# halajun/VDO_SLAM

Measured on AMD Instinct MI355X. Metric: frames/sec (per-frame hot path, KITTI-0000-shaped 1242x375) + ms/LM-iter (batch factor graph), higher is better.
Workload: dtype f64 (LM, RANSAC) / u8,i32,f32 (front-end, tracking)

## Files before the change

vdo_slam_amd/csrc/near_flags.hpp:

```cpp
#pragma once
#include <hip/hip_runtime.h>
#include <stdint.h>

namespace vdo {

static __global__ __launch_bounds__(256) void k_near_flags(int nq, const float* __restrict__ qx, const float* __restrict__ qy,
                                                           int nr, const float* __restrict__ rx, const float* __restrict__ ry, int32_t* __restrict__ used) {
  __shared__ float sx[256], sy[256];
  const int i = blockIdx.x * 256 + threadIdx.x;
  const int base = blockIdx.y * 256;
  const int j = base + threadIdx.x;
  sx[threadIdx.x] = j < nr ? rx[j] : 1e30f;
  sy[threadIdx.x] = j < nr ? ry[j] : 1e30f;
  __syncthreads();
  if (i >= nq) return;
  const float x = qx[i], y = qy[i];
  const int m = min(256, nr - base);
  int u = 0;
  for (int k = 0; k < m; ++k) {
    const float dx = sx[k] - x, dy = sy[k] - y;
    if (dx * dx + dy * dy < 1.0f) u = 1;
  }
  if (u) atomicOr(&used[i], 1);
}

static __global__ __launch_bounds__(256) void k_near_flags_sel(int nq, const float* __restrict__ qx, const float* __restrict__ qy,
                                                               int nr, const float* __restrict__ rx, const float* __restrict__ ry,
                                                               const int32_t* __restrict__ rsel, int as_int, int32_t* __restrict__ used) {
  __shared__ float sx[256], sy[256];
  const int i = blockIdx.x * 256 + threadIdx.x;
  const int base = blockIdx.y * 256;
  const int j = base + threadIdx.x;
  float vx = 1e30f, vy = 1e30f;
  if (j < nr && rsel[j]) { vx = rx[j]; vy = ry[j]; if (as_int) { vx = (float)(int)vx; vy = (float)(int)vy; } }
  sx[threadIdx.x] = vx; sy[threadIdx.x] = vy;
  __syncthreads();
  if (i >= nq) return;
  const float x = qx[i], y = qy[i];
  const int m = min(256, nr - base);
  int u = 0;
  for (int k = 0; k < m; ++k) {
    const float dx = sx[k] - x, dy = sy[k] - y;
    if (dx * dx + dy * dy < 1.0f) u = 1;
  }
  if (u) atomicOr(&used[i], 1);
}
static inline void launch_near_flags_sel(hipStream_t s, int nq, const float* qx, const float* qy, int nr, const float* rx, const float* ry, const int32_t* rsel, int as_int, int32_t* used,
                                         bool zero = true) {
  if (zero) hipMemsetAsync(used, 0, sizeof(int32_t) * (size_t)nq, s);
  if (nq > 0 && nr > 0) hipLaunchKernelGGL(k_near_flags_sel, dim3((nq + 255) / 256, (nr + 255) / 256), dim3(256), 0, s, nq, qx, qy, nr, rx, ry, rsel, as_int, used);
}

static inline void launch_near_flags(hipStream_t s, int nq, const float* qx, const float* qy, int nr, const float* rx, const float* ry, int32_t* used) {
  hipMemsetAsync(used, 0, sizeof(int32_t) * (size_t)nq, s);
  if (nq > 0 && nr > 0) hipLaunchKernelGGL(k_near_flags, dim3((nq + 255) / 256, (nr + 255) / 256), dim3(256), 0, s, nq, qx, qy, nr, rx, ry, used);
}

}
```

vdo_slam_amd/csrc/tracking.hip:

```cpp
#include <algorithm>
#include <cstring>
#include <vector>

#include "../../include/vdo_slam_hip.h"
#include "ctx.hpp"
#include "frame_images.hpp"
#include "near_flags.hpp"
#include "arena.hpp"
#include "tracking_shared.hpp"

namespace vdo {

__global__ void k_gather(int mode, int n, const float* __restrict__ kx, const float* __restrict__ ky, const float* __restrict__ depth,
                         const int32_t* __restrict__ mask, int w, int h, float th, float* __restrict__ dout, int32_t* __restrict__ lout) {
  const int i = blockIdx.x * blockDim.x + threadIdx.x;
  if (i >= n) return;
  const int u = (int)kx[i], v = (int)ky[i];
  if (mode == 0) {
    float o = -1.f;
    if (u < (w - 1) && u > 0 && v < (h - 1) && v > 0) { const float d = depth[(size_t)v * w + u]; if (d > 0) o = d; }
    dout[i] = o;
  } else if (mode == 1) {
    float o = 0.1f; int l = 0;
    if (u < (w - 1) && u > 0 && v < (h - 1) && v > 0) {
      const float d = depth[(size_t)v * w + u];
      if (d < th && d > 0) { o = d; l = mask[(size_t)v * w + u]; }
    }
    dout[i] = o; lout[i] = l;
  } else {
    lout[i] = (u < w && u > 0 && v < h && v > 0) ? mask[(size_t)v * w + u] : -1;
  }
}


__global__ void k_get3d_world(int n, const float* __restrict__ kx, const float* __restrict__ ky, const float* __restrict__ d, Cam c, float* __restrict__ xyz) {
  const int i = blockIdx.x * blockDim.x + threadIdx.x;
  if (i >= n) return;
  float o[3];
  backproject(c, kx[i], ky[i], d[i], o);
  xyz[3 * i] = o[0]; xyz[3 * i + 1] = o[1]; xyz[3 * i + 2] = o[2];
}

__global__ void k_scene_flow(int n, const float* __restrict__ cx_, const float* __restrict__ cy_, const float* __restrict__ cd, const int32_t* __restrict__ cl, Cam cc,
                             const float* __restrict__ lx, const float* __restrict__ ly, const float* __restrict__ ld, const int32_t* __restrict__ ll, Cam lc,
                             float* __restrict__ flow3d, int32_t* __restrict__ objlab) {
  const int i = blockIdx.x * blockDim.x + threadIdx.x;
  if (i >= n) return;
  if (cl[i] <= 0 || ll[i] <= 0) { objlab[i] = -1; flow3d[3 * i] = 0; flow3d[3 * i + 1] = 0; flow3d[3 * i + 2] = 0; return; }
  float p[3], c[3];
  backproject(lc, lx[i], ly[i], ld[i], p);
  backproject(cc, cx_[i], cy_[i], cd[i], c);
  flow3d[3 * i] = c[0] - p[0]; flow3d[3 * i + 1] = c[1] - p[1]; flow3d[3 * i + 2] = c[2] - p[2];
}

__global__ void k_renew_pred(int n, const float* __restrict__ px, const float* __restrict__ py, const int32_t* __restrict__ mask,
                             const float* __restrict__ depth, const float* __restrict__ flow, int w, int h,
                             int32_t* __restrict__ ok, float* __restrict__ fx, float* __restrict__ fy, float* __restrict__ dout) {
  const int i = blockIdx.x * blockDim.x + threadIdx.x;
  if (i >= n) return;
  const float x_ = px[i], y_ = py[i];
  const int x = (int)x_, y = (int)y_;
  int good = 0;
  float fxe = 0, fye = 0, d = -1.f;
  if (!(x >= w || y >= h || x <= 0 || y <= 0)) {
    const size_t o = (size_t)y * w + x;
    const float dd = depth[o];
    if (mask[o] == 0 && !(dd > 40 || dd <= 0)) {
      fxe = flow[2 * o]; fye = flow[2 * o + 1];
      if (fxe != 0 && fye != 0 && x_ + fxe < w && y_ + fye < h && x_ + fxe > 0 && y_ + fye > 0) { good = 1; d = dd > 0 ? dd : -1.f; }
    }
  }
  ok[i] = good; fx[i] = fxe; fy[i] = fye; dout[i] = d;
}

__global__ __launch_bounds__(1024) void k_carry_select(int n, const int32_t* __restrict__ ok, int max_keep, int32_t* __restrict__ sel) {
  __shared__ int lds[17];
  int carry = 0;
  for (int base = 0; base < n; base += 1024) {
    const int i = base + threadIdx.x;
    const int v = (i < n && ok[i]) ? 1 : 0;
    const int lane = threadIdx.x & 63, wv = threadIdx.x >> 6;
    int incl = v;
#pragma unroll
    for (int off = 1; off < 64; off <<= 1) { const int t = __shfl_up(incl, off, 64); if (lane >= off) incl += t; }
    __syncthreads();
    if (lane == 63) lds[wv] = incl;
    __syncthreads();
    if (threadIdx.x == 0) { int a = 0; for (int q = 0; q < 16; ++q) { const int t = lds[q]; lds[q] = a; a += t; } lds[16] = a; }
    __syncthreads();
    const int rank = carry + lds[wv] + incl - v;
    if (i < n) sel[i] = (v && rank <= max_keep) ? 1 : 0;
    carry += lds[16];
    __syncthreads();
  }
}

__global__ void k_mask_warp(const int32_t* __restrict__ mask_last, const float* __restrict__ flow_last, int w, int h, int32_t lab, int32_t* __restrict__ mask_cur) {
  const int k = blockIdx.x * blockDim.x + threadIdx.x, j = blockIdx.y;
  if (k >= w) return;
  const size_t o = (size_t)j * w + k;
  if (mask_last[o] != lab) return;
  const int fx = (int)flow_last[2 * o], fy = (int)flow_last[2 * o + 1];
  if (k + fx < w && k + fx > 0 && j + fy < h && j + fy > 0) mask_cur[(size_t)(j + fy) * w + (k + fx)] = lab;
}

}

using namespace vdo;

extern "C" int vdo_propagate_static(vdo_frame_images* f, int n, const float* kx, const float* ky, float* depth_out) {
  if (!f || n < 0) return set_error(VDO_ERR_INVALID, "bad argument");
  if (n == 0) return VDO_OK;
  int rc = ctx_bind(f->ctx);
  if (rc != VDO_OK) return rc;
  Arena S(f->ctx);
  if (!S.reserve(Arena::bytes_for(3 * (size_t)n))) return set_error(VDO_ERR_OOM, "scratch arena: allocation failed");
  float *dx = S.up(kx, n), *dy = S.up(ky, n), *dd = S.up<float>(nullptr, n);
  if (!dd) return set_error(VDO_ERR_OOM, "hipMalloc failed");
  hipLaunchKernelGGL(k_gather, dim3((n + 255) / 256), dim3(256), 0, S.stream(), 0, n, (const float*)dx, (const float*)dy, (const float*)f->d_depth, (const int32_t*)f->d_mask, f->w, f->h, 0.f, dd, (int32_t*)nullptr);
  S.down(depth_out, dd, n);
  return S.finish("vdo_propagate_static");
}

extern "C" int vdo_propagate_object(vdo_frame_images* f, int n, const float* kx, const float* ky, float th_depth_obj, float* depth_out, int32_t* label_out) {
  if (!f || n < 0) return set_error(VDO_ERR_INVALID, "bad argument");
  if (n == 0) return VDO_OK;
  int rc = ctx_bind(f->ctx);
  if (rc != VDO_OK) return rc;
  Arena S(f->ctx);
  if (!S.reserve(Arena::bytes_for(4 * (size_t)n))) return set_error(VDO_ERR_OOM, "scratch arena: allocation failed");
  float *dx = S.up(kx, n), *dy = S.up(ky, n), *dd = S.up<float>(nullptr, n);
  int32_t* dl = S.up<int32_t>(nullptr, n);
  if (!dl) return set_error(VDO_ERR_OOM, "hipMalloc failed");
  hipLaunchKernelGGL(k_gather, dim3((n + 255) / 256), dim3(256), 0, S.stream(), 1, n, (const float*)dx, (const float*)dy, (const float*)f->d_depth, (const int32_t*)f->d_mask, f->w, f->h, th_depth_obj, dd, dl);
  S.down(depth_out, dd, n); S.down(label_out, dl, n);
  return S.finish("vdo_propagate_object");
}

extern "C" int vdo_mask_at(vdo_frame_images* f, int n, const float* cx, const float* cy, int32_t* label_out) {
  if (!f || n < 0) return set_error(VDO_ERR_INVALID, "bad argument");
  if (n == 0) return VDO_OK;
  int rc = ctx_bind(f->ctx);
  if (rc != VDO_OK) return rc;
  Arena S(f->ctx);
  if (!S.reserve(Arena::bytes_for(3 * (size_t)n))) return set_error(VDO_ERR_OOM, "scratch arena: allocation failed");
  float *dx = S.up(cx, n), *dy = S.up(cy, n);
  int32_t* dl = S.up<int32_t>(nullptr, n);
  if (!dl) return set_error(VDO_ERR_OOM, "hipMalloc failed");
  hipLaunchKernelGGL(k_gather, dim3((n + 255) / 256), dim3(256), 0, S.stream(), 2, n, (const float*)dx, (const float*)dy, (const float*)f->d_depth, (const int32_t*)f->d_mask, f->w, f->h, 0.f, (float*)nullptr, dl);
  S.down(label_out, dl, n);
  return S.finish("vdo_mask_at");
}

extern "C" int vdo_mask_warp(vdo_frame_images* cur, vdo_frame_images* last, int32_t label) {
  if (!cur || !last || cur->w != last->w || cur->h != last->h) return set_error(VDO_ERR_INVALID, "bad argument");
  int rc = ctx_bind(cur->ctx);
  if (rc != VDO_OK) return rc;
  hipLaunchKernelGGL(k_mask_warp, dim3((cur->w + 255) / 256, cur->h), dim3(256), 0, cur->ctx->stream, (const int32_t*)last->d_mask, (const float*)last->d_flow, cur->w, cur->h, label, cur->d_mask);
  return VDO_OK;
}

extern "C" int vdo_frame_images_download_mask(vdo_frame_images* f, int32_t* mask_out) {
  if (!f || !mask_out) return set_error(VDO_ERR_INVALID, "bad argument");
  int rc = ctx_bind(f->ctx);
  if (rc != VDO_OK) return rc;
  hipMemcpyAsync(mask_out, f->d_mask, 4 * (size_t)f->w * f->h, hipMemcpyDeviceToHost, f->ctx->stream);
  hipError_t e = hipStreamSynchronize(f->ctx->stream);
  if (e == hipSuccess) e = hipGetLastError();
  if (e != hipSuccess) return set_error(VDO_ERR_NO_DEVICE, "vdo_frame_images_download_mask: %s", hipGetErrorString(e));
  return VDO_OK;
}

extern "C" int vdo_frame_images_download_depth(vdo_frame_images* f, float* depth_out) {
  if (!f || !depth_out) return set_error(VDO_ERR_INVALID, "bad argument");
  int rc = ctx_bind(f->ctx);
  if (rc != VDO_OK) return rc;
  hipMemcpyAsync(depth_out, f->d_depth, 4 * (size_t)f->w * f->h, hipMemcpyDeviceToHost, f->ctx->stream);
  hipError_t e = hipStreamSynchronize(f->ctx->stream);
  if (e == hipSuccess) e = hipGetLastError();
  if (e != hipSuccess) return set_error(VDO_ERR_NO_DEVICE, "vdo_frame_images_download_depth: %s", hipGetErrorString(e));
  return VDO_OK;
}

extern "C" int vdo_frame_images_download_flow(vdo_frame_images* f, float* flow_out) {
  if (!f || !flow_out) return set_error(VDO_ERR_INVALID, "bad argument");
  int rc = ctx_bind(f->ctx);
  if (rc != VDO_OK) return rc;
  hipMemcpyAsync(flow_out, f->d_flow, 8 * (size_t)f->w * f->h, hipMemcpyDeviceToHost, f->ctx->stream);
  hipError_t e = hipStreamSynchronize(f->ctx->stream);
  if (e == hipSuccess) e = hipGetLastError();
  if (e != hipSuccess) return set_error(VDO_ERR_NO_DEVICE, "vdo_frame_images_download_flow: %s", hipGetErrorString(e));
  return VDO_OK;
}

extern "C" int vdo_get3d_world(vdo_ctx* ctx, int n, const float* kx, const float* ky, const float* depth, const float K4[4], const float Twc[16], float* xyz_out) {
  if (!ctx || n < 0) return set_error(VDO_ERR_INVALID, "bad argument");
  if (n == 0) return VDO_OK;
  int rc = ctx_bind(ctx);
  if (rc != VDO_OK) return rc;
  Arena S(ctx);
  if (!S.reserve(Arena::bytes_for(6 * (size_t)n))) return set_error(VDO_ERR_OOM, "scratch arena: allocation failed");
  float *dx = S.up(kx, n), *dy = S.up(ky, n), *dd = S.up(depth, n), *dxyz = S.up<float>(nullptr, 3 * (size_t)n);
  if (!dxyz) return set_error(VDO_ERR_OOM, "hipMalloc failed");
  hipLaunchKernelGGL(k_get3d_world, dim3((n + 255) / 256), dim3(256), 0, S.stream(), n, (const float*)dx, (const float*)dy, (const float*)dd, make_cam_Twc(K4, Twc), dxyz);
  S.down(xyz_out, dxyz, 3 * (size_t)n);
  return S.finish("vdo_get3d_world");
}

extern "C" int vdo_scene_flow(vdo_ctx* ctx, int n, const float* cur_x, const float* cur_y, const float* cur_d, const int32_t* cur_label, const float Tcw_cur[16],
                              const float* last_x, const float* last_y, const float* last_d, const int32_t* last_label, const float Tcw_last[16],
                              const float K4[4], float* flow3d_out, int32_t* obj_label_inout) {
  if (!ctx || n < 0) return set_error(VDO_ERR_INVALID, "bad argument");
  if (n == 0) return VDO_OK;
  int rc = ctx_bind(ctx);
  if (rc != VDO_OK) return rc;
  Arena S(ctx);
  if (!S.reserve(Arena::bytes_for(12 * (size_t)n))) return set_error(VDO_ERR_OOM, "scratch arena: allocation failed");
  float *a = S.up(cur_x, n), *b = S.up(cur_y, n), *c = S.up(cur_d, n), *d = S.up(last_x, n), *e = S.up(last_y, n), *g = S.up(last_d, n);
  int32_t *cl = S.up(cur_label, n), *ll = S.up(last_label, n), *ol = S.up(obj_label_inout, n);
  float* fl = S.up<float>(nullptr, 3 * (size_t)n);
  if (!fl) return set_error(VDO_ERR_OOM, "hipMalloc failed");
  hipLaunchKernelGGL(k_scene_flow, dim3((n + 255) / 256), dim3(256), 0, S.stream(), n, (const float*)a, (const float*)b, (const float*)c, (const int32_t*)cl, make_cam_Tcw(K4, Tcw_cur),
                     (const float*)d, (const float*)e, (const float*)g, (const int32_t*)ll, make_cam_Tcw(K4, Tcw_last), fl, ol);
  S.down(flow3d_out, fl, 3 * (size_t)n); S.down(obj_label_inout, ol, n);
  return S.finish("vdo_scene_flow");
}

namespace {
struct K9Args { float th_depth; int32_t* keep_idx; float *corr_x, *corr_y, *flow_x, *flow_y, *depth; int* n_out; };
}
static int renew_static_world_impl(vdo_frame_images* f, int n_tm, const int32_t* tm_sta, const float* stat_x, const float* stat_y,
                                   int n_orb, const float* orb_x, const float* orb_y, int max_num_sta, const float K4[4], const float Twc[16],
                                   float* key_x, float* key_y, float* corr_x, float* corr_y, float* flow_x, float* flow_y,
                                   int32_t* inlier_id, float* depth_out, float* xyz_out, int* n_out, const K9Args* k9) {
  if (!f || !n_out || n_tm < 0 || n_orb < 0 || (xyz_out && (!K4 || !Twc))) return set_error(VDO_ERR_INVALID, "bad argument");
  if (k9 && (!k9->n_out || 10 * (size_t)n_orb > 8 * (size_t)f->cap)) return set_error(VDO_ERR_INVALID, "bad argument / too many keypoints for the staging buffer");
  if (k9) *k9->n_out = 0;
  if (k9 && n_orb == 0) k9 = nullptr;
  int rc = ctx_bind(f->ctx);
  if (rc != VDO_OK) return rc;
  Arena S(f->ctx);
  if (!S.reserve(Arena::bytes_for(24 * ((size_t)n_tm + (size_t)n_orb) + 4 * (size_t)max_num_sta + (k9 ? 6 * (size_t)n_orb + 512 : 0)))) return set_error(VDO_ERR_OOM, "scratch arena: allocation failed");
  std::vector<float> cx1, cy1; std::vector<int32_t> id1;
  for (int i = 0; i < n_tm; ++i) if (tm_sta[i] != -1) { cx1.push_back(stat_x[tm_sta[i]]); cy1.push_back(stat_y[tm_sta[i]]); id1.push_back(tm_sta[i]); }
  const int n1 = (int)cx1.size();
  std::vector<int32_t> ok1(n1), ok2(n_orb), used2(n_orb, 0);
  std::vector<float> fx1(n1), fy1(n1), d1(n1), fx2(n_orb), fy2(n_orb), d2(n_orb), xyz1(xyz_out ? 3 * (size_t)n1 : 0), xyz2(xyz_out ? 3 * (size_t)n_orb : 0);
  float *dx1 = S.up(cx1.data(), n1), *dy1 = S.up(cy1.data(), n1);
  float *dx2 = S.up(orb_x, n_orb), *dy2 = S.up(orb_y, n_orb);
  int32_t *dok1 = S.up<int32_t>(nullptr, n1), *dsel1 = S.up<int32_t>(nullptr, n1);
  float *dfx1 = S.up<float>(nullptr, n1), *dfy1 = S.up<float>(nullptr, n1), *dd1 = S.up<float>(nullptr, n1), *dxyz1 = S.up<float>(nullptr, xyz_out ? 3 * (size_t)n1 : 0);
  int32_t *dok2 = S.up<int32_t>(nullptr, n_orb), *dused = S.up<int32_t>(nullptr, n_orb);
  float *dfx2 = S.up<float>(nullptr, n_orb), *dfy2 = S.up<float>(nullptr, n_orb), *dd2 = S.up<float>(nullptr, n_orb), *dxyz2 = S.up<float>(nullptr, xyz_out ? 3 * (size_t)n_orb : 0);
  if (!dxyz2 || !dxyz1 || !dd2 || !dd1) return set_error(VDO_ERR_OOM, "scratch arena: allocation failed");
  hipStream_t s = S.stream();
  const int32_t* k9_idx = nullptr; const float* k9_row[5] = {nullptr, nullptr, nullptr, nullptr, nullptr}; const int* k9_cnt = nullptr;
  if (k9) {
    int32_t* oi = S.out<int32_t>(n_orb);
    float* orow[5];
    for (float*& r : orow) r = S.out<float>(n_orb);
    int* oc = S.out<int>(1);
    if (!oi || !orow[0] || !orow[1] || !orow[2] || !orow[3] || !orow[4] || !oc) return set_error(VDO_ERR_OOM, "scratch arena: allocation failed");
    static_filter_launch(f, s, n_orb, dx2, dy2, k9->th_depth, 0, oi, orow[0], orow[1], orow[2], orow[3], orow[4], oc);
    k9_idx = S.view(oi, n_orb); k9_cnt = S.view(oc, 1);
    for (int k = 0; k < 5; ++k) k9_row[k] = S.view(orow[k], n_orb);
  }
  const Cam cam = xyz_out ? make_cam_Twc(K4, Twc) : Cam{};
  if (n1) {
    hipLaunchKernelGGL(k_renew_pred, dim3((n1 + 255) / 256), dim3(256), 0, s, n1, (const float*)dx1, (const float*)dy1, (const int32_t*)f->d_mask, (const float*)f->d_depth, (const float*)f->d_flow, f->w, f->h, dok1, dfx1, dfy1, dd1);
    hipLaunchKernelGGL(k_carry_select, dim3(1), dim3(1024), 0, s, n1, (const int32_t*)dok1, max_num_sta, dsel1);
    if (xyz_out) hipLaunchKernelGGL(k_backproject_pts, dim3((n1 + 255) / 256), dim3(256), 0, s, n1, (const float*)dx1, (const float*)dy1, (const float*)dd1, cam, 0, dxyz1);
  }
  if (n_orb) {
    hipLaunchKernelGGL(k_renew_pred, dim3((n_orb + 255) / 256), dim3(256), 0, s, n_orb, (const float*)dx2, (const float*)dy2, (const int32_t*)f->d_mask, (const float*)f->d_depth, (const float*)f->d_flow, f->w, f->h, dok2, dfx2, dfy2, dd2);
    launch_near_flags_sel(s, n_orb, dx2, dy2, n1, dx1, dy1, dsel1, 0, dused);
    if (xyz_out) hipLaunchKernelGGL(k_backproject_pts, dim3((n_orb + 255) / 256), dim3(256), 0, s, n_orb, (const float*)dx2, (const float*)dy2, (const float*)dd2, cam, 0, dxyz2);
  }
  S.down(ok1.data(), dok1, n1); S.down(fx1.data(), dfx1, n1); S.down(fy1.data(), dfy1, n1); S.down(d1.data(), dd1, n1);
  S.down(used2.data(), dused, n_orb); S.down(ok2.data(), dok2, n_orb); S.down(fx2.data(), dfx2, n_orb); S.down(fy2.data(), dfy2, n_orb); S.down(d2.data(), dd2, n_orb);
  if (xyz_out) { S.down(xyz1.data(), dxyz1, 3 * (size_t)n1); S.down(xyz2.data(), dxyz2, 3 * (size_t)n_orb); }
  rc = S.finish("vdo_renew_static");
  if (rc != VDO_OK) return rc;
  if (k9) {
    if (!k9_idx || !k9_cnt || !k9_row[4]) return set_error(VDO_ERR_OOM, "scratch arena: allocation failed");
    const int m9 = *k9_cnt;
    *k9->n_out = m9;
    if (m9) {
      float* dst[5] = {k9->corr_x, k9->corr_y, k9->flow_x, k9->flow_y, k9->depth};
      for (int k = 0; k < 5; ++k) std::memcpy(dst[k], k9_row[k], 4 * (size_t)m9);
      std::memcpy(k9->keep_idx, k9_idx, 4 * (size_t)m9);
    }
  }
  int m = 0;
  for (int i = 0; i < n1; ++i) {
    if (ok1[i]) {
      key_x[m] = cx1[i]; key_y[m] = cy1[i]; corr_x[m] = cx1[i] + fx1[i]; corr_y[m] = cy1[i] + fy1[i];
      flow_x[m] = fx1[i]; flow_y[m] = fy1[i]; inlier_id[m] = id1[i]; depth_out[m] = d1[i];
      if (xyz_out) { xyz_out[3 * m] = xyz1[3 * i]; xyz_out[3 * m + 1] = xyz1[3 * i + 1]; xyz_out[3 * m + 2] = xyz1[3 * i + 2]; }
      ++m;
    }
    if (m > max_num_sta) break;
  }
  if (m < max_num_sta && n_orb) {
    int tot = m, start_id = 0;
    const int step = 20;
    while (tot < max_num_sta) {
      if (start_id == step) break;
      for (int i = start_id; i < n_orb; i += step) {
        if (used2[i]) continue;
        if (ok2[i]) {
          key_x[m] = orb_x[i]; key_y[m] = orb_y[i]; corr_x[m] = orb_x[i] + fx2[i]; corr_y[m] = orb_y[i] + fy2[i];
          flow_x[m] = fx2[i]; flow_y[m] = fy2[i]; inlier_id[m] = -1; depth_out[m] = d2[i];
          if (xyz_out) { xyz_out[3 * m] = xyz2[3 * i]; xyz_out[3 * m + 1] = xyz2[3 * i + 1]; xyz_out[3 * m + 2] = xyz2[3 * i + 2]; }
          ++m; ++tot;
        }
        if (tot >= max_num_sta) break;
      }
      ++start_id;
    }
  }
  *n_out = m;
  return VDO_OK;
}

extern "C" int vdo_renew_static_world(vdo_frame_images* f, int n_tm, const int32_t* tm_sta, const float* stat_x, const float* stat_y,
                                      int n_orb, const float* orb_x, const float* orb_y, int max_num_sta, const float K4[4], const float Twc[16],
                                      float* key_x, float* key_y, float* corr_x, float* corr_y, float* flow_x, float* flow_y,
                                      int32_t* inlier_id, float* depth_out, float* xyz_out, int* n_out) {
  return renew_static_world_impl(f, n_tm, tm_sta, stat_x, stat_y, n_orb, orb_x, orb_y, max_num_sta, K4, Twc, key_x, key_y, corr_x, corr_y, flow_x, flow_y,
                                 inlier_id, depth_out, xyz_out, n_out, nullptr);
}

extern "C" int vdo_static_stage(vdo_frame_images* f, int n_orb, const float* orb_x, const float* orb_y, float th_depth,
                                int32_t* keep_idx, float* s_corr_x, float* s_corr_y, float* s_flow_x, float* s_flow_y, float* s_depth, int* n_static,
                                int n_tm, const int32_t* tm_sta, const float* stat_x, const float* stat_y, int max_num_sta, const float K4[4], const float Twc[16],
                                float* key_x, float* key_y, float* corr_x, float* corr_y, float* flow_x, float* flow_y,
                                int32_t* inlier_id, float* depth_out, float* xyz_out, int* n_out) {
  if (!n_static) return set_error(VDO_ERR_INVALID, "vdo_static_stage: bad argument");
  const K9Args k9{th_depth, keep_idx, s_corr_x, s_corr_y, s_flow_x, s_flow_y, s_depth, n_static};
  return renew_static_world_impl(f, n_tm, tm_sta, stat_x, stat_y, n_orb, orb_x, orb_y, max_num_sta, K4, Twc, key_x, key_y, corr_x, corr_y, flow_x, flow_y,
                                 inlier_id, depth_out, xyz_out, n_out, &k9);
}

extern "C" int vdo_renew_static(vdo_frame_images* f, int n_tm, const int32_t* tm_sta, const float* stat_x, const float* stat_y,
                                int n_orb, const float* orb_x, const float* orb_y, int max_num_sta,
                                float* key_x, float* key_y, float* corr_x, float* corr_y, float* flow_x, float* flow_y,
                                int32_t* inlier_id, float* depth_out, int* n_out) {
  return vdo_renew_static_world(f, n_tm, tm_sta, stat_x, stat_y, n_orb, orb_x, orb_y, max_num_sta, nullptr, nullptr,
                                key_x, key_y, corr_x, corr_y, flow_x, flow_y, inlier_id, depth_out, nullptr, n_out);
}
```

vdo_slam_amd/csrc/tracking_logic.hip:

```cpp
#include <algorithm>
#include <chrono>
#include <cmath>
#include <cstring>
#include <vector>

#include "../../include/vdo_slam_hip.h"
#include "ctx.hpp"
#include "frame_images.hpp"
#include "near_flags.hpp"
#include "arena.hpp"
#include "tracking_shared.hpp"

namespace vdo {

__global__ void k_renew_obj_pred(int n, const float* __restrict__ px, const float* __restrict__ py, const int32_t* __restrict__ mask,
                                 const float* __restrict__ depth, const float* __restrict__ flow, int w, int h,
                                 int32_t* __restrict__ ok, int32_t* __restrict__ sem, float* __restrict__ dout, float* __restrict__ fx, float* __restrict__ fy) {
  const int i = blockIdx.x * blockDim.x + threadIdx.x;
  if (i >= n) return;
  const int x = (int)px[i], y = (int)py[i];
  int good = 0, sl = 0;
  float d = 0, fxe = 0, fye = 0;
  if (!(x >= w || y >= h || x <= 0 || y <= 0)) {
    const size_t o = (size_t)y * w + x;
    sl = mask[o]; d = depth[o];
    if (sl != 0 && d < 25 && d > 0) {
      fxe = flow[2 * o]; fye = flow[2 * o + 1];
      if (x + fxe < w && y + fye < h && x + fxe > 0 && y + fye > 0) good = 1;
    }
  }
  ok[i] = good; sem[i] = sl; dout[i] = d; fx[i] = fxe; fy[i] = fye;
}

__global__ void k_renew_obj_all(int n, const float* __restrict__ px, const float* __restrict__ py, const int32_t* __restrict__ mask,
                                const float* __restrict__ depth, const float* __restrict__ flow, int w, int h,
                                int32_t* __restrict__ ok, int32_t* __restrict__ sem, float* __restrict__ dout, float* __restrict__ fx, float* __restrict__ fy,
                                Cam cam, float* __restrict__ xyz_c,
                                int n_tmp, const float* __restrict__ qx, const float* __restrict__ qy, const float* __restrict__ qd, float* __restrict__ xyz_t,
                                int32_t* __restrict__ used) {
  const int i = blockIdx.x * blockDim.x + threadIdx.x;
  if (i < n) {
    const int x = (int)px[i], y = (int)py[i];
    int good = 0, sl = 0;
    float d = 0, fxe = 0, fye = 0;
    if (!(x >= w || y >= h || x <= 0 || y <= 0)) {
      const size_t o = (size_t)y * w + x;
      sl = mask[o]; d = depth[o];
      if (sl != 0 && d < 25 && d > 0) {
        fxe = flow[2 * o]; fye = flow[2 * o + 1];
        if (x + fxe < w && y + fye < h && x + fxe > 0 && y + fye > 0) good = 1;
      }
    }
    ok[i] = good; sem[i] = sl; dout[i] = d; fx[i] = fxe; fy[i] = fye;
    float o3[3];
    backproject(cam, (float)x, (float)y, d, o3);
    xyz_c[3 * i] = o3[0]; xyz_c[3 * i + 1] = o3[1]; xyz_c[3 * i + 2] = o3[2];
  }
  if (i < n_tmp) {
    used[i] = 0;
    float o3[3];
    backproject(cam, qx[i], qy[i], qd[i], o3);
    xyz_t[3 * i] = o3[0]; xyz_t[3 * i + 1] = o3[1]; xyz_t[3 * i + 2] = o3[2];
  }
}

constexpr int kVoteBins = 1024;

__global__ __launch_bounds__(256) void k_label_vote(int n, const float* __restrict__ cx, const float* __restrict__ cy,
                                                    const int32_t* __restrict__ mask, int w, int h, int32_t* __restrict__ flag) {
  __shared__ int hist[kVoteBins];
  __shared__ int s_valid, s_bad;
  for (int i = threadIdx.x; i < kVoteBins; i += 256) hist[i] = 0;
  if (threadIdx.x == 0) { s_valid = 0; s_bad = 0; }
  __syncthreads();
  for (int i = threadIdx.x; i < n; i += 256) {
    const int u = (int)cx[i], v = (int)cy[i];
    if (u < w && u > 0 && v < h && v > 0) {
      const int l = mask[(size_t)v * w + u];
      if (l < 0 || l >= kVoteBins) atomicOr(&s_bad, 1);
      else { atomicAdd(&hist[l], 1); atomicAdd(&s_valid, 1); }
    }
  }
  __syncthreads();
  __shared__ int s_cnt[256], s_lab[256];
  {
    int best = threadIdx.x * 4, cnt = hist[best];
    for (int l = best + 1; l < threadIdx.x * 4 + 4; ++l) if (hist[l] > cnt) { cnt = hist[l]; best = l; }
    s_cnt[threadIdx.x] = cnt; s_lab[threadIdx.x] = best;
  }
  __syncthreads();
  for (int step = 128; step > 0; step >>= 1) {
    if (threadIdx.x < step) {
      const int c2 = s_cnt[threadIdx.x + step], l2 = s_lab[threadIdx.x + step];
      if (c2 > s_cnt[threadIdx.x] || (c2 == s_cnt[threadIdx.x] && l2 < s_lab[threadIdx.x])) { s_cnt[threadIdx.x] = c2; s_lab[threadIdx.x] = l2; }
    }
    __syncthreads();
  }
  if (threadIdx.x == 0) {
    flag[0] = (s_valid >= 100 && s_lab[0] == 0 && !s_bad) ? 1 : 0;
    flag[1] = s_bad;
  }
}

__global__ void k_mask_warp_if(const int32_t* __restrict__ flag, const int32_t* __restrict__ mask_last, const float* __restrict__ flow_last,
                               int w, int h, int32_t lab, int32_t* __restrict__ mask_cur) {
  if (!flag[0]) return;
  const int k = blockIdx.x * blockDim.x + threadIdx.x, j = blockIdx.y;
  if (k >= w) return;
  const size_t o = (size_t)j * w + k;
  if (mask_last[o] != lab) return;
  const int fx = (int)flow_last[2 * o], fy = (int)flow_last[2 * o + 1];
  if (k + fx < w && k + fx > 0 && j + fy < h && j + fy > 0) mask_cur[(size_t)(j + fy) * w + (k + fx)] = lab;
}

// ... 197 lines not shown
  for (int i = 0; i < n; ++i) {
    if (obj_label_inout[i] == -1) continue;
    const int s = slot[i];
    ++cnt[s];
    const float u = key_x[i], v = key_y[i];
    if (v < prm->shrink_row || v > (prm->img_h - prm->shrink_row) || u < prm->shrink_col || u > (prm->img_w - prm->shrink_col)) border[s] += 1.f;
  }
  std::vector<int> state(L, 0);
  for (int s = 0; s < L; ++s) if (border[s] / (float)cnt[s] > 0.5f) state[s] = 1;
  std::vector<float> dsum(L, 0.f), slow(L, 0.f);
  for (int i = 0; i < n; ++i) {
    if (obj_label_inout[i] == -1) continue;
    const int s = slot[i];
    if (state[s] == 1) { obj_label_inout[i] = -1; continue; }
    dsum[s] = dsum[s] + depth[i];
    const float fx = flow3d[3 * i], fz = flow3d[3 * i + 2];
    if (std::sqrt(fx * fx + fz * fz) < prm->sf_mg_thres) slow[s] = slow[s] + 1.f;
  }
  for (int s = 0; s < L; ++s) {
    if (state[s]) continue;
    if (slow[s] / (float)cnt[s] > prm->sf_ds_thres) state[s] = 2;
    else if (dsum[s] / (float)cnt[s] > prm->th_depth_obj || cnt[s] < 150) state[s] = 3;
  }
  std::vector<int> acc_of(L, -1);
  int n_acc = 0;
  obj_off[0] = 0;
  for (int s = 0; s < L; ++s) if (state[s] == 0) { acc_of[s] = n_acc; obj_off[n_acc + 1] = obj_off[n_acc] + cnt[s]; obj_sem[n_acc] = uni[s]; ++n_acc; }
  std::vector<int> cur(n_acc + 1);
  for (int a = 0; a <= n_acc; ++a) cur[a] = obj_off[a];
  for (int i = 0; i < n; ++i) {
    if (obj_label_inout[i] == -1) continue;
    const int s = slot[i];
    if (state[s] == 2) obj_label_inout[i] = 0;
    else if (state[s] == 3) obj_label_inout[i] = -1;
    else if (state[s] == 0) obj_idx[cur[acc_of[s]]++] = i;
  }
  int max_id = *max_id_inout;
  if (prm->f_id == 1) max_id = 1;
  std::vector<int32_t> votes;
  for (int a = 0; a < n_acc; ++a) {
    votes.clear();
    for (int q = obj_off[a]; q < obj_off[a + 1]; ++q) votes.push_back(last_sem_label[obj_idx[q]]);
    const int new_lab = majority(votes);
    int lab = -1;
    if (max_id != 1)
      for (int k = 0; k < n_last_obj; ++k)
        if (last_sem_pos[k] == new_lab && last_obj_stat[k]) { lab = last_mod_label[k]; break; }
    if (lab == -1) { lab = max_id; max_id = max_id + 1; }
    for (int q = obj_off[a]; q < obj_off[a + 1]; ++q) obj_label_inout[obj_idx[q]] = lab;
    obj_mod[a] = lab;
  }
  *max_id_inout = max_id;
  *n_obj_out = n_acc;
  return VDO_OK;
}

extern "C" int vdo_renew_object_world(vdo_frame_images* f, int n_obj, const int32_t* inl_off, const int32_t* inl_idx, const uint8_t* obj_stat,
                                      const int32_t* sem_pos, const int32_t* mod_label,
                                      const float* cur_x, const float* cur_y, const int32_t* cur_obj_label,
                                      int n_tmp, const float* tmp_x, const float* tmp_y, const float* tmp_depth, const int32_t* tmp_label,
                                      const float* tmp_flow_x, const float* tmp_flow_y, const float* tmp_corr_x, const float* tmp_corr_y,
                                      int max_num_obj, int cap, const float K4[4], const float Twc[16],
                                      float* key_x, float* key_y, float* depth_out, int32_t* sem_out, float* flow_x, float* flow_y,
                                      float* corr_x, float* corr_y, int32_t* dyn_inlier_id, int32_t* obj_label_out, float* xyz_out, int* n_out) {
  if (!f || !n_out || n_obj < 0 || n_tmp < 0 || cap < 0 || (xyz_out && (!K4 || !Twc))) return set_error(VDO_ERR_INVALID, "vdo_renew_object: bad argument");
  int rc = ctx_bind(f->ctx);
  if (rc != VDO_OK) return rc;
  Arena S(f->ctx);
  if (!S.reserve(Arena::bytes_for(24 * ((size_t)(n_obj ? inl_off[n_obj] : 0) + (size_t)n_tmp + 64)))) return set_error(VDO_ERR_OOM, "scratch arena: allocation failed");
  static thread_local std::vector<float> cx, cy, dd, fx, fy, xyz_c, xyz_t;
  static thread_local std::vector<int32_t> cid, cobj, ok, sem, used;
  cx.clear(); cy.clear(); cid.clear(); cobj.clear();
  for (int i = 0; i < n_obj; ++i) {
    if (!obj_stat[i]) continue;
    for (int q = inl_off[i]; q < inl_off[i + 1]; ++q) { const int id = inl_idx[q]; cx.push_back(cur_x[id]); cy.push_back(cur_y[id]); cid.push_back(id); cobj.push_back(i); }
  }
  const int nc = (int)cx.size();
  ok.resize(nc); sem.resize(nc); dd.resize(nc); fx.resize(nc); fy.resize(nc);
  used.assign(n_tmp, 0);
  xyz_c.resize(xyz_out ? 3 * (size_t)nc : 0); xyz_t.resize(xyz_out ? 3 * (size_t)n_tmp : 0);
  if (nc || (n_tmp && xyz_out)) {
    float *dx = S.up(cx.data(), nc), *dy = S.up(cy.data(), nc);
    float *dqx = S.up(tmp_x, n_tmp), *dqy = S.up(tmp_y, n_tmp), *dqd = S.up(xyz_out ? tmp_depth : nullptr, xyz_out ? n_tmp : 0);
    int32_t *dok = S.up<int32_t>(nullptr, nc), *dsem = S.up<int32_t>(nullptr, nc);
    float *ddd = S.up<float>(nullptr, nc), *dfx = S.up<float>(nullptr, nc), *dfy = S.up<float>(nullptr, nc);
    int32_t* dused = S.up<int32_t>(nullptr, n_tmp);
    float *dxc = S.up<float>(nullptr, xyz_out ? 3 * (size_t)nc : 0), *dxt = S.up<float>(nullptr, xyz_out ? 3 * (size_t)n_tmp : 0);
    if (!dxt || !dxc || !dused || !dfy) return set_error(VDO_ERR_OOM, "scratch arena: allocation failed");
    hipStream_t st = S.stream();
    const Cam cam = xyz_out ? make_cam_Twc(K4, Twc) : Cam{};
    if (xyz_out) {
      const int nmax = std::max(nc, n_tmp);
      hipLaunchKernelGGL(k_renew_obj_all, dim3((nmax + 255) / 256), dim3(256), 0, st, nc, (const float*)dx, (const float*)dy, (const int32_t*)f->d_mask,
                         (const float*)f->d_depth, (const float*)f->d_flow, f->w, f->h, dok, dsem, ddd, dfx, dfy, cam, dxc,
                         n_tmp, (const float*)dqx, (const float*)dqy, (const float*)dqd, dxt, dused);
      if (nc && n_tmp) launch_near_flags_sel(st, n_tmp, dqx, dqy, nc, dx, dy, dok, 1, dused, false);
    } else if (nc) {
      hipLaunchKernelGGL(k_renew_obj_pred, dim3((nc + 255) / 256), dim3(256), 0, st, nc, (const float*)dx, (const float*)dy, (const int32_t*)f->d_mask,
                         (const float*)f->d_depth, (const float*)f->d_flow, f->w, f->h, dok, dsem, ddd, dfx, dfy);
      if (n_tmp) launch_near_flags_sel(st, n_tmp, dqx, dqy, nc, dx, dy, dok, 1, dused);
    }
    S.down(ok.data(), dok, nc); S.down(sem.data(), dsem, nc); S.down(dd.data(), ddd, nc); S.down(fx.data(), dfx, nc); S.down(fy.data(), dfy, nc);
    if (nc && n_tmp) S.down(used.data(), dused, n_tmp);
    if (xyz_out) { S.down(xyz_c.data(), dxc, 3 * (size_t)nc); S.down(xyz_t.data(), dxt, 3 * (size_t)n_tmp); }
    rc = S.finish("vdo_renew_object");
    if (rc != VDO_OK) return rc;
  }
  int m = 0;
  auto push = [&](float x, float y, float d, int sl, float flx, float fly, float crx, float cry, int inl, int ol, const float* p3) -> bool {
    if (m >= cap) return false;
    key_x[m] = x; key_y[m] = y; depth_out[m] = d; sem_out[m] = sl; flow_x[m] = flx; flow_y[m] = fly; corr_x[m] = crx; corr_y[m] = cry;
    dyn_inlier_id[m] = inl; obj_label_out[m] = ol;
    if (xyz_out) { xyz_out[3 * m] = p3[0]; xyz_out[3 * m + 1] = p3[1]; xyz_out[3 * m + 2] = p3[2]; }
    ++m;
    return true;
  };
  std::vector<int> fea_count(n_obj, -1);
  for (int i = 0; i < n_obj; ++i) if (obj_stat[i]) fea_count[i] = 0;
  for (int k = 0; k < nc; ++k) {
    if (!ok[k]) continue;
    const int x = (int)cx[k], y = (int)cy[k];
    if (!push((float)x, (float)y, dd[k], sem[k], fx[k], fy[k], x + fx[k], y + fy[k], cid[k], cur_obj_label[cid[k]], xyz_c.data() + 3 * (size_t)k)) return set_error(VDO_ERR_INVALID, "vdo_renew_object: output capacity %d too small", cap);
    ++fea_count[cobj[k]];
  }
  for (int i = 0; i < n_obj; ++i) {
    if (!obj_stat[i]) continue;
    int tot = fea_count[i];
    for (int start = 0; start < 15 && tot < max_num_obj; ++start) {
      for (int j = start; j < n_tmp; j += 15) {
        if (tmp_label[j] != sem_pos[i] || used[j]) continue;
        if (!push(tmp_x[j], tmp_y[j], tmp_depth[j], tmp_label[j], tmp_flow_x[j], tmp_flow_y[j], tmp_corr_x[j], tmp_corr_y[j], -1, mod_label[i], xyz_t.data() + 3 * (size_t)j))
          return set_error(VDO_ERR_INVALID, "vdo_renew_object: output capacity %d too small", cap);
        if (++tot >= max_num_obj) break;
      }
    }
  }
  std::vector<int32_t> uni, slot;
  label_slots(n_tmp, tmp_label, uni, slot);
  std::vector<char> known(uni.size(), 0);
  for (int i = 0; i < n_obj; ++i) {
    if (!obj_stat[i]) continue;
    auto it = std::lower_bound(uni.begin(), uni.end(), sem_pos[i]);
    if (it != uni.end() && *it == sem_pos[i]) known[it - uni.begin()] = 1;
  }
  for (size_t s = 0; s < uni.size(); ++s) {
    if (known[s]) continue;
    for (int j = 0; j < n_tmp; ++j)
      if (slot[j] == (int)s && !push(tmp_x[j], tmp_y[j], tmp_depth[j], tmp_label[j], tmp_flow_x[j], tmp_flow_y[j], tmp_corr_x[j], tmp_corr_y[j], -1, -2, xyz_t.data() + 3 * (size_t)j))
        return set_error(VDO_ERR_INVALID, "vdo_renew_object: output capacity %d too small", cap);
  }
  *n_out = m;
  return VDO_OK;
}

extern "C" int vdo_renew_object(vdo_frame_images* f, int n_obj, const int32_t* inl_off, const int32_t* inl_idx, const uint8_t* obj_stat,
                                const int32_t* sem_pos, const int32_t* mod_label,
                                const float* cur_x, const float* cur_y, const int32_t* cur_obj_label,
                                int n_tmp, const float* tmp_x, const float* tmp_y, const float* tmp_depth, const int32_t* tmp_label,
                                const float* tmp_flow_x, const float* tmp_flow_y, const float* tmp_corr_x, const float* tmp_corr_y,
                                int max_num_obj, int cap,
                                float* key_x, float* key_y, float* depth_out, int32_t* sem_out, float* flow_x, float* flow_y,
                                float* corr_x, float* corr_y, int32_t* dyn_inlier_id, int32_t* obj_label_out, int* n_out) {
  return vdo_renew_object_world(f, n_obj, inl_off, inl_idx, obj_stat, sem_pos, mod_label, cur_x, cur_y, cur_obj_label, n_tmp, tmp_x, tmp_y, tmp_depth, tmp_label,
                                tmp_flow_x, tmp_flow_y, tmp_corr_x, tmp_corr_y, max_num_obj, cap, nullptr, nullptr,
                                key_x, key_y, depth_out, sem_out, flow_x, flow_y, corr_x, corr_y, dyn_inlier_id, obj_label_out, nullptr, n_out);
}

extern "C" int vdo_update_mask(vdo_frame_images* cur, vdo_frame_images* last, int n, const int32_t* last_sem_label,
                               const float* last_corr_x, const float* last_corr_y, int* n_recovered) {
  if (!cur || !last || cur->w != last->w || cur->h != last->h || n < 0) return set_error(VDO_ERR_INVALID, "vdo_update_mask: bad argument");
  if (n_recovered) *n_recovered = 0;
  if (n == 0) return VDO_OK;
  int rc = ctx_bind(cur->ctx);
  if (rc != VDO_OK) return rc;
// ... 340 lines not shown
```

Before: 1439.

## Fuse renew predicate, carry-select and near-flag test into single-launch kernels

Adds one-launch kernels for static and object feature renewal. Each block recomputes the predicate and prefix-scan selection for all carried points into LDS, then tests its 64-query slice against the selected list, writing ok/flow/depth/xyz outputs directly. This removes several kernel launches, the memset, the global atomics and the intermediate uploads, and uses S.out output slots. In exchange every block redundantly recomputes predicates for all carried points, and the path is capped at 4096 carried points with env-var overrides. Host vectors are also made thread_local to avoid reallocation.

```diff
diff --git a/vdo_slam_amd/csrc/near_flags.hpp b/vdo_slam_amd/csrc/near_flags.hpp
--- a/vdo_slam_amd/csrc/near_flags.hpp
+++ b/vdo_slam_amd/csrc/near_flags.hpp
@@ -2,7 +2,15 @@
 #include <hip/hip_runtime.h>
 #include <stdint.h>
 
+#include <algorithm>
+#include <cstdlib>
+
 namespace vdo {
+
+__device__ __forceinline__ bool near_1px(float rx, float ry, float qx, float qy) {
+  const float dx = rx - qx, dy = ry - qy;
+  return dx * dx + dy * dy < 1.0f;
+}
 
 static __global__ __launch_bounds__(256) void k_near_flags(int nq, const float* __restrict__ qx, const float* __restrict__ qy,
                                                            int nr, const float* __restrict__ rx, const float* __restrict__ ry, int32_t* __restrict__ used) {
@@ -18,8 +26,7 @@
   const int m = min(256, nr - base);
   int u = 0;
   for (int k = 0; k < m; ++k) {
-    const float dx = sx[k] - x, dy = sy[k] - y;
-    if (dx * dx + dy * dy < 1.0f) u = 1;
+    if (near_1px(sx[k], sy[k], x, y)) u = 1;
   }
   if (u) atomicOr(&used[i], 1);
 }
@@ -40,8 +47,7 @@
   const int m = min(256, nr - base);
   int u = 0;
   for (int k = 0; k < m; ++k) {
-    const float dx = sx[k] - x, dy = sy[k] - y;
-    if (dx * dx + dy * dy < 1.0f) u = 1;
+    if (near_1px(sx[k], sy[k], x, y)) u = 1;
   }
   if (u) atomicOr(&used[i], 1);
 }
@@ -56,4 +62,26 @@
   if (nq > 0 && nr > 0) hipLaunchKernelGGL(k_near_flags, dim3((nq + 255) / 256, (nr + 255) / 256), dim3(256), 0, s, nq, qx, qy, nr, rx, ry, used);
 }
 
+constexpr int kRenewThreads = 1024, kRenewSlice = 64, kRenewCap = 4096;
+
+__device__ __forceinline__ void near_slice(const float2* list, int n, bool has_query, float x, float y, int* s_used) {
+  const int lane = threadIdx.x & 63, wv = threadIdx.x >> 6;
+  const int per = (n + kRenewThreads / 64 - 1) / (kRenewThreads / 64);
+  const int k0 = min(n, wv * per), k1 = min(n, k0 + per);
+  int u = 0;
+  for (int k = k0; k < k1; ++k) {
+    const float2 r = list[k];
+    if (near_1px(r.x, r.y, x, y)) u = 1;
+  }
+  if (u && has_query) atomicOr(&s_used[lane], 1);
 }
+
+static inline int renew_one_cap() {
+  if (std::getenv("VDO_RENEW_UNFUSED") != nullptr) return -1;
+  int cap = kRenewCap;
+  if (const char* e = std::getenv("VDO_RENEW_LDS_CAP")) cap = std::min(std::max(std::atoi(e), 0), kRenewCap);
+  return cap;
+}
+static inline int renew_one_grid(int n_carried, int n_query) { return std::max(1, (std::max(n_carried, n_query) + kRenewSlice - 1) / kRenewSlice); }
+
+}
diff --git a/vdo_slam_amd/csrc/tracking.hip b/vdo_slam_amd/csrc/tracking.hip
--- a/vdo_slam_amd/csrc/tracking.hip
+++ b/vdo_slam_amd/csrc/tracking.hip
@@ -53,15 +53,11 @@
   flow3d[3 * i] = c[0] - p[0]; flow3d[3 * i + 1] = c[1] - p[1]; flow3d[3 * i + 2] = c[2] - p[2];
 }
 
-__global__ void k_renew_pred(int n, const float* __restrict__ px, const float* __restrict__ py, const int32_t* __restrict__ mask,
-                             const float* __restrict__ depth, const float* __restrict__ flow, int w, int h,
-                             int32_t* __restrict__ ok, float* __restrict__ fx, float* __restrict__ fy, float* __restrict__ dout) {
-  const int i = blockIdx.x * blockDim.x + threadIdx.x;
-  if (i >= n) return;
-  const float x_ = px[i], y_ = py[i];
+__device__ __forceinline__ int renew_pred(float x_, float y_, const int32_t* __restrict__ mask, const float* __restrict__ depth, const float* __restrict__ flow,
+                                          int w, int h, float& fxe, float& fye, float& d) {
   const int x = (int)x_, y = (int)y_;
   int good = 0;
-  float fxe = 0, fye = 0, d = -1.f;
+  fxe = 0; fye = 0; d = -1.f;
   if (!(x >= w || y >= h || x <= 0 || y <= 0)) {
     const size_t o = (size_t)y * w + x;
     const float dd = depth[o];
@@ -70,6 +66,16 @@
       if (fxe != 0 && fye != 0 && x_ + fxe < w && y_ + fye < h && x_ + fxe > 0 && y_ + fye > 0) { good = 1; d = dd > 0 ? dd : -1.f; }
     }
   }
+  return good;
+}
+
+__global__ void k_renew_pred(int n, const float* __restrict__ px, const float* __restrict__ py, const int32_t* __restrict__ mask,
+                             const float* __restrict__ depth, const float* __restrict__ flow, int w, int h,
+                             int32_t* __restrict__ ok, float* __restrict__ fx, float* __restrict__ fy, float* __restrict__ dout) {
+  const int i = blockIdx.x * blockDim.x + threadIdx.x;
+  if (i >= n) return;
+  float fxe, fye, d;
+  const int good = renew_pred(px[i], py[i], mask, depth, flow, w, h, fxe, fye, d);
   ok[i] = good; fx[i] = fxe; fy[i] = fye; dout[i] = d;
 }
 
@@ -95,6 +101,68 @@
   }
 }
 
+__global__ __launch_bounds__(kRenewThreads) void k_renew_static_one(int n1, const float* __restrict__ px1, const float* __restrict__ py1,
+                                                                    int n2, const float* __restrict__ px2, const float* __restrict__ py2,
+                                                                    const int32_t* __restrict__ mask, const float* __restrict__ depth, const float* __restrict__ flow, int w, int h,
+                                                                    int max_keep, int has_xyz, Cam cam,
+                                                                    int32_t* __restrict__ ok1, float* __restrict__ fx1, float* __restrict__ fy1, float* __restrict__ d1, float* __restrict__ xyz1,
+                                                                    int32_t* __restrict__ ok2, int32_t* __restrict__ used2, float* __restrict__ fx2, float* __restrict__ fy2,
+                                                                    float* __restrict__ d2, float* __restrict__ xyz2) {
+  __shared__ float2 s_key[kRenewCap];
+  __shared__ float s_xyz1[3 * kRenewSlice], s_xyz2[3 * kRenewSlice];
+  __shared__ int s_used[kRenewSlice];
+  __shared__ int lds[17];
+  const int t = threadIdx.x, lane = t & 63, wv = t >> 6;
+  const int lo = blockIdx.x * kRenewSlice;
+  if (t < kRenewSlice) s_used[t] = 0;
+  int carry = 0;
+  for (int base = 0; base < n1; base += kRenewThreads) {
+    const int i = base + t;
+    int v = 0;
+    float x_ = 0, y_ = 0;
+    if (i < n1) {
+      x_ = px1[i]; y_ = py1[i];
+      float fxe, fye, d;
+      v = renew_pred(x_, y_, mask, depth, flow, w, h, fxe, fye, d);
+      if (i >= lo && i < lo + kRenewSlice) {
+        ok1[i] = v; fx1[i] = fxe; fy1[i] = fye; d1[i] = d;
+        if (has_xyz) backproject(cam, x_, y_, d, &s_xyz1[3 * (i - lo)]);
+      }
+    }
+    int incl = v;
+#pragma unroll
+    for (int off = 1; off < 64; off <<= 1) { const int u = __shfl_up(incl, off, 64); if (lane >= off) incl += u; }
+    __syncthreads();
+    if (lane == 63) lds[wv] = incl;
+    __syncthreads();
+    if (t == 0) { int a = 0; for (int q = 0; q < kRenewThreads / 64; ++q) { const int u = lds[q]; lds[q] = a; a += u; } lds[16] = a; }
+    __syncthreads();
+    const int rank = carry + lds[wv] + incl - v;
+    if (v && rank <= max_keep) s_key[rank] = make_float2(x_, y_);
+    carry += lds[16];
+    __syncthreads();
+  }
+  const int nsel = max_keep < 0 ? 0 : (carry <= max_keep ? carry : max_keep + 1);
+  const int q = lo + lane;
+  const bool has_q = q < n2;
+  float x = 0, y = 0;
+  if (has_q) { x = px2[q]; y = py2[q]; }
+  if (wv == 0 && has_q) {
+    float fxe, fye, d;
+    ok2[q] = renew_pred(x, y, mask, depth, flow, w, h, fxe, fye, d);
+    fx2[q] = fxe; fy2[q] = fye; d2[q] = d;
+    if (has_xyz) backproject(cam, x, y, d, &s_xyz2[3 * lane]);
+  }
+  near_slice(s_key, nsel, has_q, x, y, s_used);
+  __syncthreads();
+  if (t < kRenewSlice && has_q) used2[q] = s_used[t];
+  if (has_xyz) {
+    const int m1 = 3 * min(max(n1 - lo, 0), kRenewSlice), m2 = 3 * min(max(n2 - lo, 0), kRenewSlice);
+    if (t < m1) xyz1[3 * (size_t)lo + t] = s_xyz1[t];
+    if (t >= 256 && t - 256 < m2) xyz2[3 * (size_t)lo + (t - 256)] = s_xyz2[t - 256];
+  }
+}
+
 __global__ void k_mask_warp(const int32_t* __restrict__ mask_last, const float* __restrict__ flow_last, int w, int h, int32_t lab, int32_t* __restrict__ mask_cur) {
   const int k = blockIdx.x * blockDim.x + threadIdx.x, j = blockIdx.y;
   if (k >= w) return;
@@ -241,18 +309,32 @@
   if (rc != VDO_OK) return rc;
   Arena S(f->ctx);
   if (!S.reserve(Arena::bytes_for(24 * ((size_t)n_tm + (size_t)n_orb) + 4 * (size_t)max_num_sta + (k9 ? 6 * (size_t)n_orb + 512 : 0)))) return set_error(VDO_ERR_OOM, "scratch arena: allocation failed");
-  std::vector<float> cx1, cy1; std::vector<int32_t> id1;
+  static thread_local std::vector<float> cx1, cy1, fx1, fy1, d1, fx2, fy2, d2, xyz1, xyz2;
+  static thread_local std::vector<int32_t> id1, ok1, ok2, used2;
+  cx1.clear(); cy1.clear(); id1.clear();
   for (int i = 0; i < n_tm; ++i) if (tm_sta[i] != -1) { cx1.push_back(stat_x[tm_sta[i]]); cy1.push_back(stat_y[tm_sta[i]]); id1.push_back(tm_sta[i]); }
   const int n1 = (int)cx1.size();
-  std::vector<int32_t> ok1(n1), ok2(n_orb), used2(n_orb, 0);
-  std::vector<float> fx1(n1), fy1(n1), d1(n1), fx2(n_orb), fy2(n_orb), d2(n_orb), xyz1(xyz_out ? 3 * (size_t)n1 : 0), xyz2(xyz_out ? 3 * (size_t)n_orb : 0);
+  ok1.resize(n1); ok2.resize(n_orb); used2.assign(n_orb, 0);
+  fx1.resize(n1); fy1.resize(n1); d1.resize(n1); fx2.resize(n_orb); fy2.resize(n_orb); d2.resize(n_orb);
+  xyz1.resize(xyz_out ? 3 * (size_t)n1 : 0); xyz2.resize(xyz_out ? 3 * (size_t)n_orb : 0);
+  const bool one = n1 <= renew_one_cap();
   float *dx1 = S.up(cx1.data(), n1), *dy1 = S.up(cy1.data(), n1);
   float *dx2 = S.up(orb_x, n_orb), *dy2 = S.up(orb_y, n_orb);
-  int32_t *dok1 = S.up<int32_t>(nullptr, n1), *dsel1 = S.up<int32_t>(nullptr, n1);
-  float *dfx1 = S.up<float>(nullptr, n1), *dfy1 = S.up<float>(nullptr, n1), *dd1 = S.up<float>(nullptr, n1), *dxyz1 = S.up<float>(nullptr, xyz_out ? 3 * (size_t)n1 : 0);
-  int32_t *dok2 = S.up<int32_t>(nullptr, n_orb), *dused = S.up<int32_t>(nullptr, n_orb);
-  float *dfx2 = S.up<float>(nullptr, n_orb), *dfy2 = S.up<float>(nullptr, n_orb), *dd2 = S.up<float>(nullptr, n_orb), *dxyz2 = S.up<float>(nullptr, xyz_out ? 3 * (size_t)n_orb : 0);
-  if (!dxyz2 || !dxyz1 || !dd2 || !dd1) return set_error(VDO_ERR_OOM, "scratch arena: allocation failed");
+  int32_t *dok1, *dsel1 = nullptr, *dok2, *dused;
+  float *dfx1, *dfy1, *dd1, *dxyz1, *dfx2, *dfy2, *dd2, *dxyz2;
+  if (!one) {
+    dok1 = S.up<int32_t>(nullptr, n1); dsel1 = S.up<int32_t>(nullptr, n1);
+    dfx1 = S.up<float>(nullptr, n1); dfy1 = S.up<float>(nullptr, n1); dd1 = S.up<float>(nullptr, n1); dxyz1 = S.up<float>(nullptr, xyz_out ? 3 * (size_t)n1 : 0);
+    dok2 = S.up<int32_t>(nullptr, n_orb); dused = S.up<int32_t>(nullptr, n_orb);
+    dfx2 = S.up<float>(nullptr, n_orb); dfy2 = S.up<float>(nullptr, n_orb); dd2 = S.up<float>(nullptr, n_orb); dxyz2 = S.up<float>(nullptr, xyz_out ? 3 * (size_t)n_orb : 0);
+    if (!dsel1) return set_error(VDO_ERR_OOM, "scratch arena: allocation failed");
+  } else {
+    dok1 = S.out<int32_t>(n1); dfx1 = S.out<float>(n1); dfy1 = S.out<float>(n1); dd1 = S.out<float>(n1); dxyz1 = S.out<float>(xyz_out ? 3 * (size_t)n1 : 0);
+    dok2 = S.out<int32_t>(n_orb); dused = S.out<int32_t>(n_orb);
+    dfx2 = S.out<float>(n_orb); dfy2 = S.out<float>(n_orb); dd2 = S.out<float>(n_orb); dxyz2 = S.out<float>(xyz_out ? 3 * (size_t)n_orb : 0);
+  }
+  if (!dx1 || !dy1 || !dx2 || !dy2 || !dok1 || !dfx1 || !dfy1 || !dd1 || !dxyz1 || !dok2 || !dused || !dfx2 || !dfy2 || !dd2 || !dxyz2)
+    return set_error(VDO_ERR_OOM, "scratch arena: allocation failed");
   hipStream_t s = S.stream();
   const int32_t* k9_idx = nullptr; const float* k9_row[5] = {nullptr, nullptr, nullptr, nullptr, nullptr}; const int* k9_cnt = nullptr;
   if (k9) {
@@ -266,12 +348,17 @@
     for (int k = 0; k < 5; ++k) k9_row[k] = S.view(orow[k], n_orb);
   }
   const Cam cam = xyz_out ? make_cam_Twc(K4, Twc) : Cam{};
-  if (n1) {
+  if (one) {
+    if (n1 || n_orb)
+      hipLaunchKernelGGL(k_renew_static_one, dim3(renew_one_grid(n1, n_orb)), dim3(kRenewThreads), 0, s, n1, (const float*)dx1, (const float*)dy1, n_orb, (const float*)dx2, (const float*)dy2,
+                         (const int32_t*)f->d_mask, (const float*)f->d_depth, (const float*)f->d_flow, f->w, f->h, max_num_sta, xyz_out ? 1 : 0, cam,
+                         dok1, dfx1, dfy1, dd1, dxyz1, dok2, dused, dfx2, dfy2, dd2, dxyz2);
+  } else if (n1) {
     hipLaunchKernelGGL(k_renew_pred, dim3((n1 + 255) / 256), dim3(256), 0, s, n1, (const float*)dx1, (const float*)dy1, (const int32_t*)f->d_mask, (const float*)f->d_depth, (const float*)f->d_flow, f->w, f->h, dok1, dfx1, dfy1, dd1);
     hipLaunchKernelGGL(k_carry_select, dim3(1), dim3(1024), 0, s, n1, (const int32_t*)dok1, max_num_sta, dsel1);
     if (xyz_out) hipLaunchKernelGGL(k_backproject_pts, dim3((n1 + 255) / 256), dim3(256), 0, s, n1, (const float*)dx1, (const float*)dy1, (const float*)dd1, cam, 0, dxyz1);
   }
-  if (n_orb) {
+  if (!one && n_orb) {
     hipLaunchKernelGGL(k_renew_pred, dim3((n_orb + 255) / 256), dim3(256), 0, s, n_orb, (const float*)dx2, (const float*)dy2, (const int32_t*)f->d_mask, (const float*)f->d_depth, (const float*)f->d_flow, f->w, f->h, dok2, dfx2, dfy2, dd2);
     launch_near_flags_sel(s, n_orb, dx2, dy2, n1, dx1, dy1, dsel1, 0, dused);
     if (xyz_out) hipLaunchKernelGGL(k_backproject_pts, dim3((n_orb + 255) / 256), dim3(256), 0, s, n_orb, (const float*)dx2, (const float*)dy2, (const float*)dd2, cam, 0, dxyz2);
diff --git a/vdo_slam_amd/csrc/tracking_logic.hip b/vdo_slam_amd/csrc/tracking_logic.hip
--- a/vdo_slam_amd/csrc/tracking_logic.hip
+++ b/vdo_slam_amd/csrc/tracking_logic.hip
@@ -13,14 +13,10 @@
 
 namespace vdo {
 
-__global__ void k_renew_obj_pred(int n, const float* __restrict__ px, const float* __restrict__ py, const int32_t* __restrict__ mask,
-                                 const float* __restrict__ depth, const float* __restrict__ flow, int w, int h,
-                                 int32_t* __restrict__ ok, int32_t* __restrict__ sem, float* __restrict__ dout, float* __restrict__ fx, float* __restrict__ fy) {
-  const int i = blockIdx.x * blockDim.x + threadIdx.x;
-  if (i >= n) return;
-  const int x = (int)px[i], y = (int)py[i];
-  int good = 0, sl = 0;
-  float d = 0, fxe = 0, fye = 0;
+__device__ __forceinline__ int renew_obj_pred(int x, int y, const int32_t* __restrict__ mask, const float* __restrict__ depth, const float* __restrict__ flow,
+                                              int w, int h, int& sl, float& d, float& fxe, float& fye) {
+  int good = 0;
+  sl = 0; d = 0; fxe = 0; fye = 0;
   if (!(x >= w || y >= h || x <= 0 || y <= 0)) {
     const size_t o = (size_t)y * w + x;
     sl = mask[o]; d = depth[o];
@@ -29,7 +25,55 @@
       if (x + fxe < w && y + fye < h && x + fxe > 0 && y + fye > 0) good = 1;
     }
   }
+  return good;
+}
+
+__global__ void k_renew_obj_pred(int n, const float* __restrict__ px, const float* __restrict__ py, const int32_t* __restrict__ mask,
+                                 const float* __restrict__ depth, const float* __restrict__ flow, int w, int h,
+                                 int32_t* __restrict__ ok, int32_t* __restrict__ sem, float* __restrict__ dout, float* __restrict__ fx, float* __restrict__ fy) {
+  const int i = blockIdx.x * blockDim.x + threadIdx.x;
+  if (i >= n) return;
+  int sl; float d, fxe, fye;
+  const int good = renew_obj_pred((int)px[i], (int)py[i], mask, depth, flow, w, h, sl, d, fxe, fye);
   ok[i] = good; sem[i] = sl; dout[i] = d; fx[i] = fxe; fy[i] = fye;
+}
+
+__global__ __launch_bounds__(kRenewThreads) void k_renew_object_one(int nc, const float* __restrict__ px, const float* __restrict__ py, const int32_t* __restrict__ mask,
+                                                                    const float* __restrict__ depth, const float* __restrict__ flow, int w, int h,
+                                                                    int32_t* __restrict__ ok, int32_t* __restrict__ sem, float* __restrict__ dout, float* __restrict__ fx, float* __restrict__ fy,
+                                                                    int has_xyz, Cam cam, float* __restrict__ xyz_c,
+                                                                    int n_tmp, const float* __restrict__ qx, const float* __restrict__ qy, const float* __restrict__ qd,
+                                                                    float* __restrict__ xyz_t, int32_t* __restrict__ used) {
+  __shared__ float2 s_key[kRenewCap];
+  __shared__ float s_xyz_c[3 * kRenewSlice], s_xyz_t[3 * kRenewSlice];
+  __shared__ int s_used[kRenewSlice];
+  const int t = threadIdx.x, lane = t & 63, wv = t >> 6;
+  const int lo = blockIdx.x * kRenewSlice;
+  if (t < kRenewSlice) s_used[t] = 0;
+  for (int i = t; i < nc; i += kRenewThreads) {
+    const int x = (int)px[i], y = (int)py[i];
+    int sl; float d, fxe, fye;
+    const int good = renew_obj_pred(x, y, mask, depth, flow, w, h, sl, d, fxe, fye);
+    s_key[i] = good ? make_float2((float)x, (float)y) : make_float2(1e30f, 1e30f);
+    if (i >= lo && i < lo + kRenewSlice) {
+      ok[i] = good; sem[i] = sl; dout[i] = d; fx[i] = fxe; fy[i] = fye;
+      if (has_xyz) backproject(cam, (float)x, (float)y, d, &s_xyz_c[3 * (i - lo)]);
+    }
+  }
+  const int q = lo + lane;
+  const bool has_q = q < n_tmp;
+  float x = 0, y = 0;
+  if (has_q) { x = qx[q]; y = qy[q]; }
+  if (wv == 0 && has_q && has_xyz) backproject(cam, x, y, qd[q], &s_xyz_t[3 * lane]);
+  __syncthreads();
+  near_slice(s_key, nc, has_q, x, y, s_used);
+  __syncthreads();
+  if (t < kRenewSlice && has_q) used[q] = s_used[t];
+  if (has_xyz) {
+    const int m1 = 3 * min(max(nc - lo, 0), kRenewSlice), m2 = 3 * min(max(n_tmp - lo, 0), kRenewSlice);
+    if (t < m1) xyz_c[3 * (size_t)lo + t] = s_xyz_c[t];
+    if (t >= 256 && t - 256 < m2) xyz_t[3 * (size_t)lo + (t - 256)] = s_xyz_t[t - 256];
+  }
 }
 
 __global__ void k_renew_obj_all(int n, const float* __restrict__ px, const float* __restrict__ py, const int32_t* __restrict__ mask,
@@ -393,14 +437,21 @@
   if (nc || (n_tmp && xyz_out)) {
     float *dx = S.up(cx.data(), nc), *dy = S.up(cy.data(), nc);
     float *dqx = S.up(tmp_x, n_tmp), *dqy = S.up(tmp_y, n_tmp), *dqd = S.up(xyz_out ? tmp_depth : nullptr, xyz_out ? n_tmp : 0);
-    int32_t *dok = S.up<int32_t>(nullptr, nc), *dsem = S.up<int32_t>(nullptr, nc);
-    float *ddd = S.up<float>(nullptr, nc), *dfx = S.up<float>(nullptr, nc), *dfy = S.up<float>(nullptr, nc);
-    int32_t* dused = S.up<int32_t>(nullptr, n_tmp);
-    float *dxc = S.up<float>(nullptr, xyz_out ? 3 * (size_t)nc : 0), *dxt = S.up<float>(nullptr, xyz_out ? 3 * (size_t)n_tmp : 0);
-    if (!dxt || !dxc || !dused || !dfy) return set_error(VDO_ERR_OOM, "scratch arena: allocation failed");
+    const bool one = nc <= renew_one_cap();
+    auto slot_i = [&](size_t n) { return one ? S.out<int32_t>(n) : S.up<int32_t>(nullptr, n); };
+    auto slot_f = [&](size_t n) { return one ? S.out<float>(n) : S.up<float>(nullptr, n); };
+    int32_t *dok = slot_i(nc), *dsem = slot_i(nc);
+    float *ddd = slot_f(nc), *dfx = slot_f(nc), *dfy = slot_f(nc);
+    int32_t* dused = slot_i(n_tmp);
+    float *dxc = slot_f(xyz_out ? 3 * (size_t)nc : 0), *dxt = slot_f(xyz_out ? 3 * (size_t)n_tmp : 0);
+    if (!dx || !dy || !dqx || !dqy || !dqd || !dok || !dsem || !ddd || !dfx || !dfy || !dused || !dxc || !dxt) return set_error(VDO_ERR_OOM, "scratch arena: allocation failed");
     hipStream_t st = S.stream();
     const Cam cam = xyz_out ? make_cam_Twc(K4, Twc) : Cam{};
-    if (xyz_out) {
+    if (one) {
+      hipLaunchKernelGGL(k_renew_object_one, dim3(renew_one_grid(nc, n_tmp)), dim3(kRenewThreads), 0, st, nc, (const float*)dx, (const float*)dy, (const int32_t*)f->d_mask,
+                         (const float*)f->d_depth, (const float*)f->d_flow, f->w, f->h, dok, dsem, ddd, dfx, dfy, xyz_out ? 1 : 0, cam, dxc,
+                         n_tmp, (const float*)dqx, (const float*)dqy, (const float*)dqd, dxt, dused);
+    } else if (xyz_out) {
       const int nmax = std::max(nc, n_tmp);
       hipLaunchKernelGGL(k_renew_obj_all, dim3((nmax + 255) / 256), dim3(256), 0, st, nc, (const float*)dx, (const float*)dy, (const int32_t*)f->d_mask,
                          (const float*)f->d_depth, (const float*)f->d_flow, f->w, f->h, dok, dsem, ddd, dfx, dfy, cam, dxc,
```

After: 1476 (median of 6 runs). +2.5%, better.
